# srndpty/kobato-eyes

Hardware: AMD Instinct MI355X
Metric: images/s (pHash + all-pairs Hamming scan + cluster membership) (higher is better)
Workload: dtype u8 luma, int32 taps (i8 matrix cores), f64 DCT, 1-bit Hamming products (fp4 matrix cores, exact)

## Files before the change

### kobato-eyes_amd/csrc/ke_api.hip

```cpp
#include <cstdarg>
#include <cstdio>
#include <algorithm>
#include <cmath>
#include <numeric>
#include <unordered_map>

#include <fcntl.h>
#include <sys/stat.h>
#include <unistd.h>

#include "ke_internal.h"

static thread_local std::string g_create_err;

int ke_fail(ke_ctx *ctx, int code, const char *fmt, ...) {
    char msg[512];
    va_list ap;
    va_start(ap, fmt);
    vsnprintf(msg, sizeof msg, fmt, ap);
    va_end(ap);
    if (ctx)
        ctx->err = msg;
    else
        g_create_err = msg;
// ... 129 lines not shown
        delete t;
        return nullptr;
    }
    c->mx[key] = t;
    return t;
}

void ke_time_begin(ke_ctx *ctx, int kind) {
    ctx->ev_valid[kind] = false;
    (void)hipEventRecord(ctx->ev0[kind], ctx->stream);
}

void ke_time_end(ke_ctx *ctx, int kind) {
    if (hipEventRecord(ctx->ev1[kind], ctx->stream) == hipSuccess) ctx->ev_valid[kind] = true;
}

KE_API int ke_abi_version(void) { return KE_ABI_VERSION; }

KE_API const char *ke_create_error(void) { return g_create_err.c_str(); }

KE_API ke_ctx *ke_create(int device_id) {
    int count = 0;
    if (hipGetDeviceCount(&count) != hipSuccess || count <= 0) {
        ke_fail(nullptr, KE_ENODEV, "no HIP device visible (libkeyes_hip has no CPU fallback)");
        return nullptr;
    }
    if (device_id < 0 || device_id >= count) {
        ke_fail(nullptr, KE_EINVAL, "device_id %d out of range [0,%d)", device_id, count);
        return nullptr;
    }
    if (hipSetDevice(device_id) != hipSuccess) {
        ke_fail(nullptr, KE_EHIP, "hipSetDevice(%d) failed", device_id);
        return nullptr;
    }
    hipDeviceProp_t prop;
    if (hipGetDeviceProperties(&prop, device_id) != hipSuccess) {
        ke_fail(nullptr, KE_EHIP, "hipGetDeviceProperties failed");
        return nullptr;
    }
    if (std::strncmp(prop.gcnArchName, "gfx950", 6) != 0) {
        ke_fail(nullptr, KE_ENODEV, "device %d is %s; this library is built for gfx950 only", device_id,
                prop.gcnArchName);
        return nullptr;
    }
    auto *ctx = new ke_ctx();
    ctx->device = device_id;
    ctx->cu_count = prop.multiProcessorCount;
    if (hipStreamCreateWithFlags(&ctx->own_stream, hipStreamNonBlocking) != hipSuccess) {
        ke_fail(nullptr, KE_EHIP, "hipStreamCreate failed");
        delete ctx;
        return nullptr;
    }
    ctx->stream = ctx->own_stream;
    for (int k = 0; k < KE_T_COUNT; ++k) {
        (void)hipEventCreate(&ctx->ev0[k]);
        (void)hipEventCreate(&ctx->ev1[k]);
    }
    return ctx;
}

static void stage_free(ke_ctx *ctx);

KE_API void ke_destroy(ke_ctx *ctx) {
    if (!ctx) return;
    (void)hipSetDevice(ctx->device);
    (void)hipStreamSynchronize(ctx->stream);
    stage_free(ctx);
    for (int k = 0; k < 2; ++k) {
        if (ctx->side[k]) (void)hipStreamDestroy(ctx->side[k]);
        if (ctx->side_join[k]) (void)hipEventDestroy(ctx->side_join[k]);
    }
    if (ctx->side_fork) (void)hipEventDestroy(ctx->side_fork);
    if (ctx->h_comm) (void)hipHostFree(ctx->h_comm);
    if (ctx->h_meta) (void)hipHostFree(ctx->h_meta);
    for (auto &b : ctx->buf)
        if (b.ptr) (void)hipFree(b.ptr);
    free_coeff_cache(ctx);
    for (int k = 0; k < KE_T_COUNT; ++k) {
        (void)hipEventDestroy(ctx->ev0[k]);
        (void)hipEventDestroy(ctx->ev1[k]);
    }
    (void)hipStreamDestroy(ctx->own_stream);
    delete ctx;
}

KE_API const char *ke_last_error(ke_ctx *ctx) { return ctx ? ctx->err.c_str() : g_create_err.c_str(); }

KE_API int ke_set_stream(ke_ctx *ctx, void *hip_stream) {
    if (!ctx) return KE_EINVAL;
    ctx->stream = hip_stream ? (hipStream_t)hip_stream : ctx->own_stream;
    return KE_OK;
}

KE_API void *ke_get_stream(ke_ctx *ctx) { return ctx ? (void *)ctx->stream : nullptr; }

KE_API int ke_synchronize(ke_ctx *ctx) {
    if (!ctx) return KE_EINVAL;
    KE_HIP(ctx, hipStreamSynchronize(ctx->stream));
    return KE_OK;
}

KE_API int ke_device_info(ke_ctx *ctx, char *name, size_t name_len, int32_t *compute_units, int64_t *total_mem) {
    if (!ctx) return KE_EINVAL;
    hipDeviceProp_t prop;
    KE_HIP(ctx, hipGetDeviceProperties(&prop, ctx->device));
    if (name && name_len) std::snprintf(name, name_len, "%s (%s)", prop.name, prop.gcnArchName);
    if (compute_units) *compute_units = prop.multiProcessorCount;
    if (total_mem) *total_mem = (int64_t)prop.totalGlobalMem;
    return KE_OK;
}

KE_API int ke_malloc(ke_ctx *ctx, size_t bytes, void **out) {
    if (!ctx || !out) return KE_EINVAL;
    KE_HIP(ctx, hipMalloc(out, bytes ? bytes : 16));
    return KE_OK;
}

KE_API int ke_free(ke_ctx *ctx, void *p) {
    if (!ctx) return KE_EINVAL;
    KE_HIP(ctx, hipStreamSynchronize(ctx->stream));
    KE_HIP(ctx, hipFree(p));
    return KE_OK;
}

KE_API int ke_host_alloc(ke_ctx *ctx, size_t bytes, void **out) {
    if (!ctx || !out) return KE_EINVAL;
    KE_HIP(ctx, hipSetDevice(ctx->device));
// ... 485 lines not shown
        }
        cursor += 2 * idx.size();
    }
    if (used) KE_HIP(ctx, hipMemcpyAsync(s.d_px, s.h_px, used, hipMemcpyHostToDevice, st->copy_stream));
    if (cursor) KE_HIP(ctx, hipMemcpyAsync(s.d_meta, s.h_meta, cursor * 8, hipMemcpyHostToDevice, st->copy_stream));
    KE_HIP(ctx, hipEventRecord(s.copied, st->copy_stream));
    KE_HIP(ctx, hipStreamWaitEvent(ctx->stream, s.copied, 0));
    if (phash_out) KE_HIP(ctx, hipMemsetAsync(s.d_ph, 0, (size_t)n * 8, ctx->stream));
    if (dhash_out) KE_HIP(ctx, hipMemsetAsync(s.d_dh, 0, (size_t)n * 8, ctx->stream));
    if (margin_out) KE_HIP(ctx, hipMemsetAsync(s.d_mg, 0, (size_t)n * 4, ctx->stream));
    MarginScope margin_scope{ctx};
    ctx->margin_cur = margin_out ? s.d_mg : nullptr;
    ke_time_begin(ctx, KE_T_HASH);
    size_t gi = 0;
    for (auto &kv : groups) {
        const int w = std::get<0>(kv.first), h = std::get<1>(kv.first), c = std::get<2>(kv.first);
        const uint64_t *d_off = s.d_meta + spans[gi].first;
        const int64_t m = (int64_t)spans[gi].second;
        KeHashGroup g{s.d_px, d_off, (uint64_t)w * h * c, (const int64_t *)(d_off + m), m, w, h, c};
        for (int64_t idx : kv.second)
            if (((uintptr_t)s.d_px + offsets[idx]) % 4 != 0) { g.misaligned = true; break; }
        KE_TRY(ke_launch_hash_group(ctx, g, phash_out ? s.d_ph : nullptr, dhash_out ? s.d_dh : nullptr, nullptr, nullptr));
        ++gi;
    }
    ke_time_end(ctx, KE_T_HASH);
    if (phash_out) KE_HIP(ctx, hipMemcpyAsync(s.h_ph, s.d_ph, (size_t)n * 8, hipMemcpyDeviceToHost, ctx->stream));
    if (dhash_out) KE_HIP(ctx, hipMemcpyAsync(s.h_dh, s.d_dh, (size_t)n * 8, hipMemcpyDeviceToHost, ctx->stream));
    if (margin_out) KE_HIP(ctx, hipMemcpyAsync(s.h_mg, s.d_mg, (size_t)n * 4, hipMemcpyDeviceToHost, ctx->stream));
    KE_HIP(ctx, hipEventRecord(s.done, ctx->stream));
    s.user_ph = phash_out; s.user_dh = dhash_out; s.user_mg = margin_out; s.n = n;
    s.in_flight = true;
    return KE_OK;
}

KE_API int ke_hamming_scan(ke_ctx *ctx, const uint64_t *hashes, const int64_t *ids, const int64_t *sizes, int64_t n,
                           int32_t part_index, int32_t part_count, int32_t threshold, int32_t band_bits,
                           int32_t band_count, double size_ratio, int64_t bucket_pair_cap, ke_edge *edges_out,
                           int64_t capacity, int64_t *n_edges_out, uint64_t *counters_out) {
    if (!ctx) return KE_EINVAL;
    if (n < 0 || (n > 0 && !hashes)) return ke_fail(ctx, KE_EINVAL, "hashes is NULL");
    if (!n_edges_out) return ke_fail(ctx, KE_EINVAL, "n_edges_out is NULL");
    if (band_bits <= 0) return ke_fail(ctx, KE_EINVAL, "band_bits must be positive");
    if (band_count <= 0) return ke_fail(ctx, KE_EINVAL, "band_count must be positive");
    if ((int64_t)band_bits * band_count > 64) return ke_fail(ctx, KE_EINVAL, "band config too large");
    if (threshold < 0 || threshold > 64) return ke_fail(ctx, KE_EINVAL, "hamming_threshold must be in [0, 64]");
    if (part_count <= 0 || part_index < 0 || part_index >= part_count)
        return ke_fail(ctx, KE_EINVAL, "bad shard %d/%d", part_index, part_count);
    if (capacity < 0 || (capacity > 0 && !edges_out)) return ke_fail(ctx, KE_EINVAL, "edges_out is NULL");
    *n_edges_out = 0;
    if (counters_out) std::memset(counters_out, 0, 4 * sizeof(uint64_t));
    if (n < 2) return KE_OK;
    KE_HIP(ctx, hipSetDevice(ctx->device));
    const void *d_h, *d_ids, *d_sizes;
    const bool any_host = !ke_is_device_ptr(hashes) || (ids && !ke_is_device_ptr(ids)) || (sizes && !ke_is_device_ptr(sizes));
    if (any_host) {
        void *base;
        KE_TRY(ke_reserve(ctx, KE_BUF_SCAN_IN, (size_t)n * 24, &base));
        auto stage = [&](const void *src, size_t slot, const void **dst) -> int {
            if (!src) { *dst = nullptr; return KE_OK; }
            if (ke_is_device_ptr(src)) { *dst = src; return KE_OK; }
            void *d = (uint8_t *)base + slot * (size_t)n * 8;
            KE_HIP(ctx, hipMemcpyAsync(d, src, (size_t)n * 8, hipMemcpyHostToDevice, ctx->stream));
            *dst = d;
            return KE_OK;
        };
        KE_TRY(stage(hashes, 0, &d_h));
        KE_TRY(stage(ids, 1, &d_ids));
        KE_TRY(stage(sizes, 2, &d_sizes));
    } else {
        d_h = hashes; d_ids = ids; d_sizes = sizes;
    }
    const bool edges_dev = capacity > 0 && ke_is_device_ptr(edges_out);
    ke_edge *d_edges = edges_out;
    void *tmp;
    if (capacity > 0 && !edges_dev) {
        KE_TRY(ke_reserve(ctx, KE_BUF_SCAN_EDGES, (size_t)capacity * sizeof(ke_edge), &tmp));
        d_edges = (ke_edge *)tmp;
    }
    KE_TRY(ke_reserve(ctx, KE_BUF_SCAN_CNT, 4 * sizeof(unsigned long long), &tmp));
    unsigned long long *d_cnt = (unsigned long long *)tmp;
    KE_HIP(ctx, hipMemsetAsync(d_cnt, 0, 4 * sizeof(unsigned long long), ctx->stream));
    unsigned long long pairs = 0;
    KE_TRY(ke_launch_scan(ctx, (const uint64_t *)d_h, (const int64_t *)d_ids, (const int64_t *)d_sizes, n, part_index,
                          part_count, threshold, band_bits, band_count, size_ratio, bucket_pair_cap, d_edges, capacity,
                          d_cnt, &pairs, counters_out != nullptr));
    unsigned long long h_cnt[4];
    KE_HIP(ctx, hipMemcpyAsync(h_cnt, d_cnt, sizeof h_cnt, hipMemcpyDeviceToHost, ctx->stream));
    KE_HIP(ctx, hipStreamSynchronize(ctx->stream));
    *n_edges_out = (int64_t)h_cnt[2];
    if (h_cnt[0] != pairs)
        return ke_fail(ctx, KE_EHIP, "scan evaluated %llu pairs, expected %llu", h_cnt[0], pairs);
    if (counters_out)
        for (int k = 0; k < 4; ++k) counters_out[k] = h_cnt[k];
    if (capacity > 0 && !edges_dev) {
        const int64_t m = std::min<int64_t>(capacity, (int64_t)h_cnt[2]);
        if (m > 0) {
            KE_HIP(ctx, hipMemcpyAsync(edges_out, d_edges, (size_t)m * sizeof(ke_edge), hipMemcpyDeviceToHost, ctx->stream));
            KE_HIP(ctx, hipStreamSynchronize(ctx->stream));
        }
    }
    return KE_OK;
}

KE_API int ke_band_pairs_after_size(ke_ctx *ctx, const uint64_t *hashes, const int64_t *sizes, int64_t n, int32_t band_bits,
                                    int32_t band_count, double size_ratio, int64_t bucket_pair_cap, uint64_t *count_out) {
    if (!ctx) return KE_EINVAL;
    if (!count_out) return ke_fail(ctx, KE_EINVAL, "count_out is NULL");
    if (n < 0 || (n > 0 && (!hashes || !sizes))) return ke_fail(ctx, KE_EINVAL, "hashes / sizes is NULL");
    if (band_bits <= 0 || band_count <= 0 || (int64_t)band_bits * band_count > 64) return ke_fail(ctx, KE_EINVAL, "bad band config");
    if (!(size_ratio > 0.0)) return ke_fail(ctx, KE_EINVAL, "size_ratio must be positive (without a size filter the counter equals the bucket pairs)");
    *count_out = 0;
    if (n < 2) return KE_OK;
    KE_HIP(ctx, hipSetDevice(ctx->device));
    const void *d_h = hashes, *d_s = sizes;
    if (!ke_is_device_ptr(hashes) || !ke_is_device_ptr(sizes)) {
        void *base;
        KE_TRY(ke_reserve(ctx, KE_BUF_SCAN_IN, (size_t)n * 24, &base));
        if (!ke_is_device_ptr(hashes)) {
            KE_HIP(ctx, hipMemcpyAsync(base, hashes, (size_t)n * 8, hipMemcpyHostToDevice, ctx->stream));
            d_h = base;
        }
        if (!ke_is_device_ptr(sizes)) {
            void *d = (uint8_t *)base + (size_t)n * 16;
            KE_HIP(ctx, hipMemcpyAsync(d, sizes, (size_t)n * 8, hipMemcpyHostToDevice, ctx->stream));
            d_s = d;
        }
    }
    void *tmp;
    KE_TRY(ke_reserve(ctx, KE_BUF_SCAN_CNT, 4 * sizeof(unsigned long long), &tmp));
    unsigned long long *d_cnt = (unsigned long long *)tmp;
    KE_HIP(ctx, hipMemsetAsync(d_cnt, 0, sizeof(unsigned long long), ctx->stream));
    KE_TRY(ke_launch_band_pairs_after_size(ctx, (const uint64_t *)d_h, (const int64_t *)d_s, n, band_bits, band_count, size_ratio,
                                           bucket_pair_cap, d_cnt));
    unsigned long long h = 0;
    KE_HIP(ctx, hipMemcpyAsync(&h, d_cnt, sizeof h, hipMemcpyDeviceToHost, ctx->stream));
    KE_HIP(ctx, hipStreamSynchronize(ctx->stream));
    *count_out = h;
    return KE_OK;
}

// ... 312 lines not shown
```

### kobato-eyes_amd/csrc/ke_internal.h

```cpp
#pragma once

#include <hip/hip_runtime.h>

#include <cstdint>
#include <cstring>
#include <map>
#include <string>
#include <thread>
#include <tuple>
#include <utility>
#include <vector>

#include "../../include/keyes.h"

#define KE_API extern "C" __attribute__((visibility("default")))

struct KeAxisCoeffs {
    int in_size = 0, out_size = 0;
    int ksize = 0;
    std::vector<int32_t> bounds;
    std::vector<int32_t> kk;
    int ndw = 0;
    int span = 0;
    std::vector<int32_t> start;
// ... 41 lines not shown
    KE_BUF_SCAN_IN,
    KE_BUF_SCAN_AUX,
    KE_BUF_SCAN_EDGES,
    KE_BUF_SCAN_CNT,
    KE_BUF_SCAN_HIST,
    KE_BUF_SCAN_EXP,
    KE_BUF_SSIM_IN,
    KE_BUF_SSIM_AUX,
    KE_BUF_COMM,
    KE_BUF_COMM_EDGES,
    KE_BUF_JPEG_TABLES,
    KE_BUF_COUNT
};

constexpr int KE_MAX_STAGE_SLOTS = 4;
struct KeStageSlot {
    uint8_t *h_px = nullptr, *d_px = nullptr;
    uint64_t *h_meta = nullptr, *d_meta = nullptr;
    uint64_t *h_ph = nullptr, *h_dh = nullptr, *d_ph = nullptr, *d_dh = nullptr;
    float *h_mg = nullptr, *d_mg = nullptr;
    hipEvent_t copied = nullptr, done = nullptr;
    bool in_flight = false;
    bool px_external = false;
    uint64_t *user_ph = nullptr, *user_dh = nullptr;
    float *user_mg = nullptr;
    int64_t n = 0;
};
struct KeStage {
    size_t bytes = 0;
    int64_t max_images = 0;
    int n_slots = 0, next = 0;
    hipStream_t copy_stream = nullptr;
    KeStageSlot slot[KE_MAX_STAGE_SLOTS];
};

struct ke_ctx {
    int device = 0;
    int cu_count = 0;
    hipStream_t own_stream = nullptr;
    hipStream_t stream = nullptr;
    std::string err;
    KeDevBuf buf[KE_BUF_COUNT];
    std::map<std::tuple<int, int, uint32_t, uint32_t>, KeAxisCoeffs *> coeffs;
    hipEvent_t ev0[KE_T_COUNT] = {}, ev1[KE_T_COUNT] = {};
    bool ev_valid[KE_T_COUNT] = {};
    KeStage *stage = nullptr;
    hipStream_t side[2] = {nullptr, nullptr};
    hipEvent_t side_fork = nullptr, side_join[2] = {nullptr, nullptr};
    int64_t edge_slots = 1024;
    void *h_comm = nullptr;
    size_t h_comm_bytes = 0;
    void *h_meta = nullptr;
    size_t h_meta_bytes = 0;
    bool ssim_exact = false;
    float *margin_cur = nullptr;
    bool dct_tables_ready = false;
};

int ke_fail(ke_ctx *ctx, int code, const char *fmt, ...);
#define KE_HIP(ctx, call)                                                                        \
    do {                                                                                         \
        hipError_t e_ = (call);                                                                  \
        if (e_ != hipSuccess)                                                                    \
            return ke_fail((ctx), KE_EHIP, "%s failed: %s (%s:%d)", #call, hipGetErrorString(e_), \
                           __FILE__, __LINE__);                                                  \
    } while (0)
#define KE_TRY(expr)            \
    do {                        \
        int rc_ = (expr);       \
        if (rc_ != KE_OK) return rc_; \
    } while (0)

bool ke_is_device_ptr(const void *p);
int ke_reserve(ke_ctx *ctx, int which, size_t bytes, void **out);
int ke_to_device(ke_ctx *ctx, const void *p, size_t bytes, int which, const void **dev);
const KeAxisCoeffs *ke_get_coeffs(ke_ctx *ctx, int in_size, int out_size, int filter = KE_FILTER_LANCZOS, float in0 = 0.0f,
                                  float in1 = -1.0f);
const KeChunkTable *ke_get_chunks(ke_ctx *ctx, const KeAxisCoeffs *c, int cpo, int ndwc_multiple = 4);
const KeMxTable *ke_get_mx(ke_ctx *ctx, const KeAxisCoeffs *c, int min_ks = 0, bool align64 = false);
void ke_time_begin(ke_ctx *ctx, int kind);
void ke_time_end(ke_ctx *ctx, int kind);

struct KeHashGroup {
    const uint8_t *pixels;
    const uint64_t *offsets;
    uint64_t stride;
    const int64_t *out_idx;
    int64_t n;
    int w, h, channels;
    bool misaligned = false;
};
int ke_launch_hash_group(ke_ctx *ctx, const KeHashGroup &g, uint64_t *d_phash, uint64_t *d_dhash,
                         uint8_t *d_tile32_out, uint8_t *d_tile98_out, hipStream_t fused_stream = nullptr);
int ke_launch_resize_group(ke_ctx *ctx, const KeHashGroup &g, int ow, int oh, int filter, uint8_t *d_tiles,
                           const float *box = nullptr);
int ke_launch_tile_ahash(ke_ctx *ctx, const uint8_t *d_tiles, int64_t n, int grid, int tile, uint64_t *d_bits);
int ke_launch_sad_pairs(ke_ctx *ctx, const uint8_t *d_thumbs, int64_t pixels, const int64_t *d_pa, const int64_t *d_pb,
                        int64_t n_pairs, uint64_t *d_out);
int ke_launch_band_pairs_after_size(ke_ctx *ctx, const uint64_t *d_hashes, const int64_t *d_sizes, int64_t n, int band_bits,
                                    int band_count, double ratio, int64_t bucket_pair_cap, unsigned long long *d_out);
int ke_launch_scan(ke_ctx *ctx, const uint64_t *d_hashes, const int64_t *d_ids, const int64_t *d_sizes, int64_t n,
                   int part_index, int part_count, int threshold, int band_bits, int band_count, double size_ratio,
                   int64_t bucket_pair_cap, ke_edge *d_edges, int64_t capacity, unsigned long long *d_counters,
                   unsigned long long *pairs_evaluated, bool want_bucket_pairs);
int ke_launch_ssim(ke_ctx *ctx, const uint8_t *d_images, int w, int h, int channels, const int64_t *d_pa,
                   const int64_t *d_pb, int64_t n_pairs, double *d_out);
// ... 16 lines not shown
```

### kobato-eyes_amd/csrc/ke_scan.hip

```cpp
#include <cmath>

#include <hipcub/hipcub.hpp>

#include "ke_internal.h"

namespace {

constexpr int kThreads = 512;
constexpr int kRT = 8;
constexpr int kTile = 8 * kRT * 16;
constexpr int kCols = 1024;
constexpr int kCPR = kTile / kCols;
constexpr int kChunk = 256;

typedef int ke_v8i __attribute__((ext_vector_type(8)));
typedef int ke_v4i __attribute__((ext_vector_type(4)));
typedef float ke_v4f __attribute__((ext_vector_type(4)));

struct ScanArgs {
    const uint64_t *hashes;
    const ke_v4i *expanded;
    const int64_t *ids;
    const int64_t *sizes;
    int64_t n;
    int nb;
    int ncc;
    int64_t first_tile;
    int64_t tile_step;
    int64_t n_tiles;
    int threshold, band_bits, band_count;
    double size_ratio;
    const uint32_t *hist;
    const uint32_t *blen;
    unsigned long long cap;
    ke_edge *edges;
    int64_t capacity;
    unsigned long long *counters;
    int xcd_remap;
};

__device__ __forceinline__ int popc64(uint32_t lo, uint32_t hi) { return __popc(lo) + __popc(hi); }

__device__ void consider_pair(const ScanArgs &a, int64_t gi, int64_t gj, uint64_t x, uint64_t y, int pc) {
    if (gi >= gj || gj >= a.n) return;
    if (a.ids && a.ids[gi] == a.ids[gj]) return;
    if (a.sizes && a.size_ratio > 0.0) {
        const int64_t sa = a.sizes[gi], sb = a.sizes[gj];
        if (sa > 0 && sb > 0) {
            const int64_t small = sa < sb ? sa : sb, large = sa < sb ? sb : sa;
            if (!((double)small / (double)large >= a.size_ratio)) return;
        }
    }
    const uint64_t d = x ^ y;
    const uint64_t mask = a.band_bits >= 64 ? ~0ull : ((1ull << a.band_bits) - 1ull);
    int bands = 0, shared = 0;
    for (int b = 0; b < a.band_count; ++b) {
        const int sh = b * a.band_bits;
        if (((d >> sh) & mask) != 0) continue;
        if (a.cap) {
            const unsigned long long len = a.hist ? a.hist[((size_t)b << a.band_bits) + (size_t)((x >> sh) & mask)]
                                                  : a.blen[(size_t)b * (size_t)a.n + (size_t)gi];
            if (len * (len - 1) / 2 > a.cap) continue;
        }
        bands |= 1 << (b < 31 ? b : 31);
        ++shared;
    }
    if (!shared) return;
    atomicAdd(&a.counters[1], (unsigned long long)shared);
    const unsigned long long slot = atomicAdd(&a.counters[2], 1ull);
    if ((int64_t)slot < a.capacity) {
        ke_edge e;
        e.a = gi; e.b = gj; e.h = pc; e.bands = bands;
        a.edges[slot] = e;
    }
}

__device__ __forceinline__ uint32_t spread8(uint32_t b) {
    uint32_t t = (b | (b << 12)) & 0x000F000Fu;
    t = (t | (t << 6)) & 0x03030303u;
    t = (t | (t << 3)) & 0x11111111u;
    return t << 1;
}

__global__ __launch_bounds__(256) void ke_scan_expand(const uint64_t *__restrict__ hashes, int64_t n, int64_t n_pad,
                                                       ke_v4i *__restrict__ out) {
    const int64_t e = (int64_t)blockIdx.x * 256 + threadIdx.x;
    if (e >= n_pad * 4) return;
    const int64_t i = (e >> 6) * 16 + (e & 15);
    const int g = (int)(e >> 4) & 3;
    ke_v4i v = {0, 0, 0, 0};
    if (i < n) {
        const uint64_t x = g < 2 ? hashes[i] : ~hashes[i];
        const uint32_t half = (uint32_t)(x >> (32 * (g & 1)));
#pragma unroll
        for (int k = 0; k < 4; ++k) v[k] = (int)spread8((half >> (8 * k)) & 0xFFu);
    }
    out[e] = v;
}

__global__ __launch_bounds__(kThreads) void ke_scan_tiles(const ScanArgs a) {
    __shared__ ke_v4i s_b[2][kChunk / 16 * 64];
    const int tid = threadIdx.x, lane = tid & 63, wv = tid >> 6;
    int64_t slot = blockIdx.x;
    if (a.xcd_remap) {
        const int64_t per = ((int64_t)gridDim.x + 7) / 8;
        slot = (int64_t)(blockIdx.x & 7) * per + (blockIdx.x >> 3);
        if (slot >= (int64_t)gridDim.x) return;
    }
    const int64_t t = a.first_tile + slot * a.tile_step;
    if (t >= a.n_tiles) return;
    const double hc = 0.5 * kCPR, bq = (double)a.ncc + hc;
    int64_t rb = (int64_t)floor((bq - sqrt(fmax(bq * bq - 4.0 * hc * (double)t, 0.0))) / (2.0 * hc));
    if (rb < 0) rb = 0;
    if (rb >= a.nb) rb = a.nb - 1;
    while (rb > 0 && rb * a.ncc - kCPR * rb * (rb - 1) / 2 > t) --rb;
    while (rb + 1 < a.nb && (rb + 1) * a.ncc - kCPR * (rb + 1) * rb / 2 <= t) ++rb;
    const int64_t cc = kCPR * rb + (t - (rb * a.ncc - kCPR * rb * (rb - 1) / 2));
    const int64_t row0 = rb * kTile, col0 = cc * kCols;
    const int64_t wrow0 = row0 + (int64_t)wv * (kRT * 16);
    if (tid == 0) {
        const int64_t rows = min((int64_t)kTile, a.n - row0), cols = min((int64_t)kCols, a.n - col0);
        const unsigned long long pairs = cc == kCPR * rb ? (unsigned long long)(rows * (rows - 1) / 2) : (unsigned long long)(rows * cols);
        atomicAdd(&a.counters[0], pairs);
    }

    ke_v8i ra[kRT];
#pragma unroll
    for (int r = 0; r < kRT; ++r) {
        const ke_v4i v = a.expanded[(wrow0 / 16 + r) * 64 + lane];
        ra[r] = ke_v8i{v[0], v[1], v[2], v[3], 0, 0, 0, 0};
    }
    const int thr_bits = __float_as_int((float)(64 - a.threshold));
    const int nchunks = (int)((min((int64_t)kCols, a.n - col0) + kChunk - 1) / kChunk);
    const ke_v4i *cbase = a.expanded + (col0 / 16) * 64;
    ke_v4i pre0 = cbase[tid], pre1 = cbase[kThreads + tid];
    s_b[0][tid] = pre0;
    s_b[0][kThreads + tid] = pre1;
    __builtin_amdgcn_s_waitcnt(0x0F70);
    __syncthreads();
    for (int c = 0; c < nchunks; ++c) {
        {
            const int cn = c + 1 < nchunks ? c + 1 : c;
            pre0 = cbase[cn * (kChunk / 16 * 64) + tid];
            pre1 = cbase[cn * (kChunk / 16 * 64) + kThreads + tid];
        }
        const ke_v4i *bt = s_b[c & 1];
        const int64_t below = wrow0 - (col0 + (int64_t)c * kChunk) - 15;
        const int ct0 = below < 0 ? 0 : (int)min((int64_t)(kChunk / 16), below / 16 + 1);
        for (int ct = ct0; ct < kChunk / 16; ++ct) {
            const ke_v4i bv = bt[ct * 64 + lane];
            const ke_v8i b = {bv[0], bv[1], bv[2], bv[3], 0, 0, 0, 0};
            ke_v4f acc[kRT];
#pragma unroll
            for (int r = 0; r < kRT; ++r)
                acc[r] = __builtin_amdgcn_mfma_scale_f32_16x16x128_f8f6f4(ra[r], b, ke_v4f{0, 0, 0, 0}, 4, 4, 0, 0, 0, 0);
            int m = 0;
#pragma unroll
            for (int r = 0; r < kRT; ++r) {
                m = max(max(m, __float_as_int(acc[r][0])), __float_as_int(acc[r][1]));
                m = max(max(m, __float_as_int(acc[r][2])), __float_as_int(acc[r][3]));
            }
            if (__ballot(m >= thr_bits) != 0ull) {
                uint32_t hits = 0;
#pragma unroll
                for (int r = 0; r < kRT; ++r)
#pragma unroll
                    for (int i = 0; i < 4; ++i) hits |= __float_as_int(acc[r][i]) >= thr_bits ? 1u << (4 * r + i) : 0u;
                const int64_t gj = col0 + (int64_t)c * kChunk + ct * 16 + (lane & 15);
                if (gj >= a.n) hits = 0;
                const uint64_t y = hits ? a.hashes[gj] : 0ull;
                while (hits) {
                    const int k = __ffs(hits) - 1;
                    hits &= hits - 1;
                    const int64_t gi = wrow0 + (k >> 2) * 16 + 4 * (lane >> 4) + (k & 3);
                    if (gi < gj) {
                        const uint64_t x = a.hashes[gi];
                        consider_pair(a, gi, gj, x, y, __popcll(x ^ y));
                    }
                }
            }
        }
        s_b[(c + 1) & 1][tid] = pre0;
        s_b[(c + 1) & 1][kThreads + tid] = pre1;
        __syncthreads();
    }
}

__global__ void ke_band_hist(const uint64_t *__restrict__ hashes, int64_t n, int band_bits, int band_count,
                             uint32_t *__restrict__ hist) {
    const int64_t i = (int64_t)blockIdx.x * blockDim.x + threadIdx.x;
    if (i >= n) return;
    const uint64_t x = hashes[i];
    const uint64_t mask = (1ull << band_bits) - 1ull;
    for (int b = 0; b < band_count; ++b) atomicAdd(&hist[((size_t)b << band_bits) + (size_t)((x >> (b * band_bits)) & mask)], 1u);
}

__global__ void ke_hist_pairs(const uint32_t *__restrict__ hist, size_t bins, unsigned long long cap, unsigned long long *out) {
    unsigned long long s = 0;
    for (size_t i = (size_t)blockIdx.x * blockDim.x + threadIdx.x; i < bins; i += (size_t)gridDim.x * blockDim.x) {
        const unsigned long long len = hist[i];
        const unsigned long long p = len * (len - 1) / 2;
        if (len >= 2 && (!cap || p <= cap)) s += p;
    }
    for (int d = 32; d > 0; d >>= 1) s += __shfl_down(s, d);
    __shared__ unsigned long long part[4];
    if ((threadIdx.x & 63) == 0) part[threadIdx.x >> 6] = s;
    __syncthreads();
    if (threadIdx.x == 0 && (part[0] | part[1] | part[2] | part[3])) atomicAdd(out, part[0] + part[1] + part[2] + part[3]);
}

__global__ void ke_band_keys(const uint64_t *__restrict__ hashes, int64_t n, int shift, uint64_t mask, uint64_t *__restrict__ keys,
                             uint32_t *__restrict__ pos) {
    const int64_t i = (int64_t)blockIdx.x * blockDim.x + threadIdx.x;
    if (i >= n) return;
    keys[i] = (hashes[i] >> shift) & mask;
    pos[i] = (uint32_t)i;
}

__global__ void ke_run_lengths(const uint64_t *__restrict__ keys, const uint32_t *__restrict__ pos, int64_t n, unsigned long long cap,
                               uint32_t *__restrict__ blen, unsigned long long *out) {
    const int64_t i = (int64_t)blockIdx.x * blockDim.x + threadIdx.x;
    if (i >= n) return;
    if (i > 0 && keys[i - 1] == keys[i]) return;
    int64_t e = i + 1;
    while (e < n && keys[e] == keys[i]) ++e;
    const unsigned long long len = (unsigned long long)(e - i);
    for (int64_t k = i; k < e; ++k) blen[pos[k]] = (uint32_t)len;
    const unsigned long long p = len * (len - 1) / 2;
    if (len >= 2 && (!cap || p <= cap)) atomicAdd(out, p);
}

__global__ void ke_size_keys(const int64_t *__restrict__ sizes, int64_t n, uint64_t *__restrict__ keys, uint32_t *__restrict__ pos) {
    const int64_t i = (int64_t)blockIdx.x * blockDim.x + threadIdx.x;
    if (i >= n) return;
    const int64_t s = sizes[i];
    keys[i] = s > 0 ? (uint64_t)s : 0ull;
    pos[i] = (uint32_t)i;
}

__global__ void ke_band_keys_of(const uint64_t *__restrict__ hashes, const uint32_t *__restrict__ order, int64_t n, int shift,
                                uint64_t mask, uint64_t *__restrict__ keys) {
    const int64_t i = (int64_t)blockIdx.x * blockDim.x + threadIdx.x;
    if (i < n) keys[i] = (hashes[order[i]] >> shift) & mask;
}

__global__ void ke_run_flags(const uint64_t *__restrict__ keys, int64_t n, uint32_t *__restrict__ flags) {
    const int64_t i = (int64_t)blockIdx.x * blockDim.x + threadIdx.x;
// ... 49 lines not shown
    KE_HIP(ctx, hipcub::DeviceRadixSort::SortPairs(nullptr, t_size, (const uint64_t *)nullptr, (uint64_t *)nullptr,
                                                   (const uint32_t *)nullptr, (uint32_t *)nullptr, (int)n, 0, 64, ctx->stream));
    KE_HIP(ctx, hipcub::DeviceRadixSort::SortPairs(nullptr, t_band, (const uint64_t *)nullptr, (uint64_t *)nullptr,
                                                   (const uint64_t *)nullptr, (uint64_t *)nullptr, (int)n, 0, band_bits, ctx->stream));
    KE_HIP(ctx, hipcub::DeviceScan::InclusiveSum(nullptr, t_scan, (const uint32_t *)nullptr, (uint32_t *)nullptr, (int)n, ctx->stream));
    const size_t temp_bytes = std::max(t_size, std::max(t_band, t_scan));
    const size_t kb = ((size_t)n * 8 + 255) & ~(size_t)255, pb = ((size_t)(n + 1) * 4 + 255) & ~(size_t)255;
    void *scratch;
    KE_TRY(ke_reserve(ctx, KE_BUF_SCAN_AUX, 4 * kb + 4 * pb + temp_bytes + 256, &scratch));
    uint8_t *sp = (uint8_t *)scratch;
    uint64_t *k_a = (uint64_t *)sp, *k_b = (uint64_t *)(sp + kb), *sz_sorted = (uint64_t *)(sp + 2 * kb), *sz_band = (uint64_t *)(sp + 3 * kb);
    uint32_t *p_a = (uint32_t *)(sp + 4 * kb), *order = (uint32_t *)(sp + 4 * kb + pb), *rank1 = (uint32_t *)(sp + 4 * kb + 2 * pb),
             *starts = (uint32_t *)(sp + 4 * kb + 3 * pb);
    void *temp = sp + 4 * kb + 4 * pb;
    const dim3 grid((unsigned)((n + 255) / 256)), blk(256);
    const uint64_t mask = band_bits >= 64 ? ~0ull : ((1ull << band_bits) - 1ull);
    hipLaunchKernelGGL(ke_size_keys, grid, blk, 0, ctx->stream, d_sizes, n, k_a, p_a);
    size_t tb = temp_bytes;
    KE_HIP(ctx, hipcub::DeviceRadixSort::SortPairs(temp, tb, (const uint64_t *)k_a, sz_sorted, (const uint32_t *)p_a, order, (int)n, 0, 64, ctx->stream));
    for (int b = 0; b < band_count; ++b) {
        hipLaunchKernelGGL(ke_band_keys_of, grid, blk, 0, ctx->stream, d_hashes, (const uint32_t *)order, n, b * band_bits, mask, k_a);
        tb = temp_bytes;
        KE_HIP(ctx, hipcub::DeviceRadixSort::SortPairs(temp, tb, (const uint64_t *)k_a, k_b, (const uint64_t *)sz_sorted, sz_band, (int)n, 0,
                                                       band_bits, ctx->stream));
        uint32_t *flags = p_a;
        hipLaunchKernelGGL(ke_run_flags, grid, blk, 0, ctx->stream, (const uint64_t *)k_b, n, flags);
        tb = temp_bytes;
        KE_HIP(ctx, hipcub::DeviceScan::InclusiveSum(temp, tb, (const uint32_t *)flags, rank1, (int)n, ctx->stream));
        hipLaunchKernelGGL(ke_run_starts, grid, blk, 0, ctx->stream, (const uint64_t *)k_b, (const uint32_t *)rank1, n, starts);
        hipLaunchKernelGGL(ke_size_pairs, grid, blk, 0, ctx->stream, (const uint64_t *)sz_band, (const uint32_t *)rank1,
                           (const uint32_t *)starts, n, ratio, cap, d_out);
        KE_HIP(ctx, hipGetLastError());
    }
    return KE_OK;
}

int ke_launch_scan(ke_ctx *ctx, const uint64_t *d_hashes, const int64_t *d_ids, const int64_t *d_sizes, int64_t n,
                   int part_index, int part_count, int threshold, int band_bits, int band_count, double size_ratio,
                   int64_t bucket_pair_cap, ke_edge *d_edges, int64_t capacity, unsigned long long *d_counters,
                   unsigned long long *pairs_evaluated, bool want_bucket_pairs) {
    ScanArgs a;
    a.hashes = d_hashes; a.ids = d_ids; a.sizes = (size_ratio > 0.0) ? d_sizes : nullptr;
    a.n = n;
    a.nb = (int)((n + kTile - 1) / kTile);
    a.ncc = (int)((n + kCols - 1) / kCols);
    a.n_tiles = (int64_t)a.nb * a.ncc - (int64_t)kCPR * a.nb * (a.nb - 1) / 2;
    a.first_tile = part_index;
    a.tile_step = part_count;
    a.threshold = threshold; a.band_bits = band_bits; a.band_count = band_count;
    a.size_ratio = size_ratio;
    a.hist = nullptr; a.blen = nullptr;
    a.cap = bucket_pair_cap > 0 ? (unsigned long long)bucket_pair_cap : 0ull;
    a.edges = d_edges; a.capacity = capacity; a.counters = d_counters;
    if ((bucket_pair_cap > 0 || want_bucket_pairs) && band_bits <= 24) {
        void *h;
        const size_t bins = (size_t)band_count << band_bits, bytes = bins * sizeof(uint32_t);
        KE_TRY(ke_reserve(ctx, KE_BUF_SCAN_HIST, bytes, &h));
        KE_HIP(ctx, hipMemsetAsync(h, 0, bytes, ctx->stream));
        hipLaunchKernelGGL(ke_band_hist, dim3((unsigned)((n + 255) / 256)), dim3(256), 0, ctx->stream, d_hashes, n, band_bits,
                           band_count, (uint32_t *)h);
        KE_HIP(ctx, hipGetLastError());
        a.hist = (const uint32_t *)h;
        if (want_bucket_pairs) {
            const unsigned blocks = (unsigned)std::min<size_t>((bins + 1023) / 1024, 256);
            hipLaunchKernelGGL(ke_hist_pairs, dim3(blocks), dim3(256), 0, ctx->stream, (const uint32_t *)h, bins, a.cap, d_counters + 3);
            KE_HIP(ctx, hipGetLastError());
        }
    } else if (bucket_pair_cap > 0 || want_bucket_pairs) {
        if (n > 0xffffffffLL) return ke_fail(ctx, KE_EUNSUPPORTED, "bands wider than 24 bits need n < 2^32");
        size_t temp_bytes = 0;
        KE_HIP(ctx, hipcub::DeviceRadixSort::SortPairs(nullptr, temp_bytes, (const uint64_t *)nullptr, (uint64_t *)nullptr,
                                                       (const uint32_t *)nullptr, (uint32_t *)nullptr, (int)n, 0, band_bits, ctx->stream));
        const size_t kb = ((size_t)n * 8 + 255) & ~(size_t)255, pb = ((size_t)n * 4 + 255) & ~(size_t)255;
        void *scratch, *lens;
        KE_TRY(ke_reserve(ctx, KE_BUF_SCAN_AUX, 2 * kb + 2 * pb + temp_bytes + 256, &scratch));
        KE_TRY(ke_reserve(ctx, KE_BUF_SCAN_HIST, (size_t)band_count * n * sizeof(uint32_t), &lens));
        uint8_t *sp = (uint8_t *)scratch;
        uint64_t *k_in = (uint64_t *)sp, *k_out = (uint64_t *)(sp + kb);
        uint32_t *p_in = (uint32_t *)(sp + 2 * kb), *p_out = (uint32_t *)(sp + 2 * kb + pb);
        void *temp = sp + 2 * kb + 2 * pb;
        const uint64_t mask = band_bits >= 64 ? ~0ull : ((1ull << band_bits) - 1ull);
        const dim3 grid((unsigned)((n + 255) / 256)), blk(256);
        for (int b = 0; b < band_count; ++b) {
            hipLaunchKernelGGL(ke_band_keys, grid, blk, 0, ctx->stream, d_hashes, n, b * band_bits, mask, k_in, p_in);
            KE_HIP(ctx, hipcub::DeviceRadixSort::SortPairs(temp, temp_bytes, k_in, k_out, p_in, p_out, (int)n, 0, band_bits, ctx->stream));
            hipLaunchKernelGGL(ke_run_lengths, grid, blk, 0, ctx->stream, k_out, p_out, n, a.cap, (uint32_t *)lens + (size_t)b * n,
                               want_bucket_pairs ? d_counters + 3 : d_counters + 3);
            KE_HIP(ctx, hipGetLastError());
        }
        a.blen = (const uint32_t *)lens;
    }
    const int64_t my_tiles = a.n_tiles > part_index ? (a.n_tiles - part_index + part_count - 1) / part_count : 0;
    const int64_t n_pad = (int64_t)a.nb * kTile;
    void *exp;
    KE_TRY(ke_reserve(ctx, KE_BUF_SCAN_EXP, (size_t)n_pad * 64, &exp));
    a.expanded = (const ke_v4i *)exp;
    ke_time_begin(ctx, KE_T_SCAN);
    if (my_tiles > 0) {
        hipLaunchKernelGGL(ke_scan_expand, dim3((unsigned)((n_pad * 4 + 255) / 256)), dim3(256), 0, ctx->stream, d_hashes, n, n_pad,
                           (ke_v4i *)exp);
        if (my_tiles > 0x7fffffffLL) return ke_fail(ctx, KE_EUNSUPPORTED, "too many tiles for one launch");
        static const int xcd = [] { const char *e = std::getenv("KE_SCAN_XCD"); return e ? std::atoi(e) : 0; }();
        a.xcd_remap = xcd;
        const int64_t grid = xcd ? (my_tiles + 7) / 8 * 8 : my_tiles;
        hipLaunchKernelGGL(ke_scan_tiles, dim3((unsigned)grid), dim3(kThreads), 0, ctx->stream, a);
        KE_HIP(ctx, hipGetLastError());
    }
    ke_time_end(ctx, KE_T_SCAN);
    unsigned long long pairs = 0;
    for (int64_t rb = 0; rb < a.nb; ++rb) {
        const int64_t off = rb * a.ncc - (int64_t)kCPR * rb * (rb - 1) / 2;
        const int64_t row0 = rb * kTile, rows = std::min<int64_t>(kTile, n - row0);
        for (int64_t cc = kCPR * rb; cc < a.ncc; ++cc) {
            const int64_t t = off + (cc - kCPR * rb);
            const bool diagonal = cc < kCPR * (rb + 1);
            if (!diagonal) {
                const int64_t last = a.ncc - 1;
                const int64_t t_last = off + (last - kCPR * rb);
                const int64_t first_full_t = t, end_full_t = t_last;
                if (end_full_t > first_full_t) {
                    auto upto = [&](int64_t x) { return x <= part_index ? 0 : (x - part_index + part_count - 1) / part_count; };
                    pairs += (unsigned long long)(upto(end_full_t) - upto(first_full_t)) * (unsigned long long)(rows * kCols);
                }
                if (t_last % part_count == part_index && last >= cc)
                    pairs += (unsigned long long)(rows * std::min<int64_t>(kCols, n - last * kCols));
                break;
            }
            if (t % part_count != part_index) continue;
            const int64_t col0 = cc * kCols, cols = std::min<int64_t>(kCols, n - col0);
            for (int64_t j = col0; j < col0 + cols; ++j)
                pairs += (unsigned long long)std::max<int64_t>(0, std::min<int64_t>(rows, j - row0));
        }
    }
    *pairs_evaluated = pairs;
    return KE_OK;
}
```

Baseline: 8.599 million.

## Switch Hamming scan to 32x32 fp4 MFMA with half-size expanded hashes

Re-encodes hash bits so that a single fp4 MFMA over 64 bits yields the Hamming distance directly, via an offset/bias encoding. This removes the separate complemented operand and halves the expanded-hash buffer. The scan now uses 32x32x64 MFMA tiles (4 row tiles of 32) instead of 16x16x128, with one prefetch per thread per chunk. The band histogram build and counter clearing are folded into the expand kernel, which drops a memset and a launch. A pinned host counter block replaces the stack readback, and a bias template variant handles thresholds of 32 and above, which adds some risk to correctness of the threshold encoding.

```diff
diff --git a/kobato-eyes_amd/csrc/ke_api.hip b/kobato-eyes_amd/csrc/ke_api.hip
--- a/kobato-eyes_amd/csrc/ke_api.hip
+++ b/kobato-eyes_amd/csrc/ke_api.hip
@@ -205,6 +205,12 @@
         return nullptr;
     }
     ctx->stream = ctx->own_stream;
+    if (hipHostMalloc((void **)&ctx->h_words, 8 * sizeof(unsigned long long), hipHostMallocDefault) != hipSuccess) {
+        ke_fail(nullptr, KE_EHIP, "hipHostMalloc of the counter block failed");
+        (void)hipStreamDestroy(ctx->own_stream);
+        delete ctx;
+        return nullptr;
+    }
     for (int k = 0; k < KE_T_COUNT; ++k) {
         (void)hipEventCreate(&ctx->ev0[k]);
         (void)hipEventCreate(&ctx->ev1[k]);
@@ -226,6 +232,7 @@
     if (ctx->side_fork) (void)hipEventDestroy(ctx->side_fork);
     if (ctx->h_comm) (void)hipHostFree(ctx->h_comm);
     if (ctx->h_meta) (void)hipHostFree(ctx->h_meta);
+    if (ctx->h_words) (void)hipHostFree(ctx->h_words);
     for (auto &b : ctx->buf)
         if (b.ptr) (void)hipFree(b.ptr);
     free_coeff_cache(ctx);
@@ -817,23 +824,20 @@
     if (n < 2) return KE_OK;
     KE_HIP(ctx, hipSetDevice(ctx->device));
     const void *d_h, *d_ids, *d_sizes;
-    const bool any_host = !ke_is_device_ptr(hashes) || (ids && !ke_is_device_ptr(ids)) || (sizes && !ke_is_device_ptr(sizes));
-    if (any_host) {
+    const bool h_dev = ke_is_device_ptr(hashes), i_dev = !ids || ke_is_device_ptr(ids), s_dev = !sizes || ke_is_device_ptr(sizes);
+    d_h = hashes; d_ids = ids; d_sizes = sizes;
+    if (!h_dev || !i_dev || !s_dev) {
         void *base;
         KE_TRY(ke_reserve(ctx, KE_BUF_SCAN_IN, (size_t)n * 24, &base));
         auto stage = [&](const void *src, size_t slot, const void **dst) -> int {
-            if (!src) { *dst = nullptr; return KE_OK; }
-            if (ke_is_device_ptr(src)) { *dst = src; return KE_OK; }
             void *d = (uint8_t *)base + slot * (size_t)n * 8;
             KE_HIP(ctx, hipMemcpyAsync(d, src, (size_t)n * 8, hipMemcpyHostToDevice, ctx->stream));
             *dst = d;
             return KE_OK;
         };
-        KE_TRY(stage(hashes, 0, &d_h));
-        KE_TRY(stage(ids, 1, &d_ids));
-        KE_TRY(stage(sizes, 2, &d_sizes));
-    } else {
-        d_h = hashes; d_ids = ids; d_sizes = sizes;
+        if (!h_dev) KE_TRY(stage(hashes, 0, &d_h));
+        if (!i_dev) KE_TRY(stage(ids, 1, &d_ids));
+        if (!s_dev) KE_TRY(stage(sizes, 2, &d_sizes));
     }
     const bool edges_dev = capacity > 0 && ke_is_device_ptr(edges_out);
     ke_edge *d_edges = edges_out;
@@ -844,13 +848,12 @@
     }
     KE_TRY(ke_reserve(ctx, KE_BUF_SCAN_CNT, 4 * sizeof(unsigned long long), &tmp));
     unsigned long long *d_cnt = (unsigned long long *)tmp;
-    KE_HIP(ctx, hipMemsetAsync(d_cnt, 0, 4 * sizeof(unsigned long long), ctx->stream));
     unsigned long long pairs = 0;
     KE_TRY(ke_launch_scan(ctx, (const uint64_t *)d_h, (const int64_t *)d_ids, (const int64_t *)d_sizes, n, part_index,
                           part_count, threshold, band_bits, band_count, size_ratio, bucket_pair_cap, d_edges, capacity,
                           d_cnt, &pairs, counters_out != nullptr));
-    unsigned long long h_cnt[4];
-    KE_HIP(ctx, hipMemcpyAsync(h_cnt, d_cnt, sizeof h_cnt, hipMemcpyDeviceToHost, ctx->stream));
+    unsigned long long *h_cnt = ctx->h_words;
+    KE_HIP(ctx, hipMemcpyAsync(h_cnt, d_cnt, 4 * sizeof(unsigned long long), hipMemcpyDeviceToHost, ctx->stream));
     KE_HIP(ctx, hipStreamSynchronize(ctx->stream));
     *n_edges_out = (int64_t)h_cnt[2];
     if (h_cnt[0] != pairs)
diff --git a/kobato-eyes_amd/csrc/ke_internal.h b/kobato-eyes_amd/csrc/ke_internal.h
--- a/kobato-eyes_amd/csrc/ke_internal.h
+++ b/kobato-eyes_amd/csrc/ke_internal.h
@@ -117,6 +117,7 @@
     size_t h_comm_bytes = 0;
     void *h_meta = nullptr;
     size_t h_meta_bytes = 0;
+    unsigned long long *h_words = nullptr;
     bool ssim_exact = false;
     float *margin_cur = nullptr;
     bool dct_tables_ready = false;
diff --git a/kobato-eyes_amd/csrc/ke_scan.hip b/kobato-eyes_amd/csrc/ke_scan.hip
--- a/kobato-eyes_amd/csrc/ke_scan.hip
+++ b/kobato-eyes_amd/csrc/ke_scan.hip
@@ -7,15 +7,16 @@
 namespace {
 
 constexpr int kThreads = 512;
-constexpr int kRT = 8;
-constexpr int kTile = 8 * kRT * 16;
+constexpr int kRT = 4;
+constexpr int kOT = 32;
+constexpr int kTile = 8 * kRT * kOT;
 constexpr int kCols = 1024;
 constexpr int kCPR = kTile / kCols;
 constexpr int kChunk = 256;
 
 typedef int ke_v8i __attribute__((ext_vector_type(8)));
 typedef int ke_v4i __attribute__((ext_vector_type(4)));
-typedef float ke_v4f __attribute__((ext_vector_type(4)));
+typedef float ke_v16f __attribute__((ext_vector_type(16)));
 
 struct ScanArgs {
     const uint64_t *hashes;
@@ -79,27 +80,34 @@
     uint32_t t = (b | (b << 12)) & 0x000F000Fu;
     t = (t | (t << 6)) & 0x03030303u;
     t = (t | (t << 3)) & 0x11111111u;
-    return t << 1;
-}
-
-__global__ __launch_bounds__(256) void ke_scan_expand(const uint64_t *__restrict__ hashes, int64_t n, int64_t n_pad,
-                                                       ke_v4i *__restrict__ out) {
+    return (t << 3) | 0x22222222u;
+}
+
+__global__ __launch_bounds__(256) void ke_scan_prepare(const uint64_t *__restrict__ hashes, int64_t n, int64_t n_pad,
+                                                        ke_v4i *__restrict__ out, int band_bits, int band_count,
+                                                        uint32_t *__restrict__ hist, unsigned long long *__restrict__ counters,
+                                                        int clear_counters) {
     const int64_t e = (int64_t)blockIdx.x * 256 + threadIdx.x;
-    if (e >= n_pad * 4) return;
-    const int64_t i = (e >> 6) * 16 + (e & 15);
-    const int g = (int)(e >> 4) & 3;
+    if (e < 4 && clear_counters) counters[e] = 0ull;
+    if (e >= n_pad * 2) return;
+    const int64_t i = (e >> 6) * kOT + (e & 31);
     ke_v4i v = {0, 0, 0, 0};
     if (i < n) {
-        const uint64_t x = g < 2 ? hashes[i] : ~hashes[i];
-        const uint32_t half = (uint32_t)(x >> (32 * (g & 1)));
+        const uint32_t half = (uint32_t)(hashes[i] >> (32 * ((int)(e >> 5) & 1)));
 #pragma unroll
         for (int k = 0; k < 4; ++k) v[k] = (int)spread8((half >> (8 * k)) & 0xFFu);
     }
     out[e] = v;
-}
-
+    if (hist && e < n) {
+        const uint64_t x = hashes[e];
+        const uint64_t mask = (1ull << band_bits) - 1ull;
+        for (int b = 0; b < band_count; ++b) atomicAdd(&hist[((size_t)b << band_bits) + (size_t)((x >> (b * band_bits)) & mask)], 1u);
+    }
+}
+
+template <bool kBias>
 __global__ __launch_bounds__(kThreads) void ke_scan_tiles(const ScanArgs a) {
-    __shared__ ke_v4i s_b[2][kChunk / 16 * 64];
+    __shared__ ke_v4i s_b[2][kChunk / kOT * 64];
     const int tid = threadIdx.x, lane = tid & 63, wv = tid >> 6;
     int64_t slot = blockIdx.x;
     if (a.xcd_remap) {
@@ -117,7 +125,7 @@
     while (rb + 1 < a.nb && (rb + 1) * a.ncc - kCPR * (rb + 1) * rb / 2 <= t) ++rb;
     const int64_t cc = kCPR * rb + (t - (rb * a.ncc - kCPR * rb * (rb - 1) / 2));
     const int64_t row0 = rb * kTile, col0 = cc * kCols;
-    const int64_t wrow0 = row0 + (int64_t)wv * (kRT * 16);
+    const int64_t wrow0 = row0 + (int64_t)wv * (kRT * kOT);
     if (tid == 0) {
         const int64_t rows = min((int64_t)kTile, a.n - row0), cols = min((int64_t)kCols, a.n - col0);
         const unsigned long long pairs = cc == kCPR * rb ? (unsigned long long)(rows * (rows - 1) / 2) : (unsigned long long)(rows * cols);
@@ -127,52 +135,56 @@
     ke_v8i ra[kRT];
 #pragma unroll
     for (int r = 0; r < kRT; ++r) {
-        const ke_v4i v = a.expanded[(wrow0 / 16 + r) * 64 + lane];
+        const ke_v4i v = a.expanded[(wrow0 / kOT + r) * 64 + lane];
         ra[r] = ke_v8i{v[0], v[1], v[2], v[3], 0, 0, 0, 0};
     }
-    const int thr_bits = __float_as_int((float)(64 - a.threshold));
+    constexpr float kStart = kBias ? 65.0f : 0.0f;
+    const int thr_bits = __float_as_int(kStart + (float)(64 - 2 * a.threshold));
     const int nchunks = (int)((min((int64_t)kCols, a.n - col0) + kChunk - 1) / kChunk);
-    const ke_v4i *cbase = a.expanded + (col0 / 16) * 64;
-    ke_v4i pre0 = cbase[tid], pre1 = cbase[kThreads + tid];
-    s_b[0][tid] = pre0;
-    s_b[0][kThreads + tid] = pre1;
+    constexpr int kPieces = kChunk / kOT * 64;
+    static_assert(kPieces == kThreads, "one piece of a column chunk per thread");
+    const ke_v4i *cbase = a.expanded + (col0 / kOT) * 64;
+    ke_v4i pre = cbase[tid];
+    s_b[0][tid] = pre;
     __builtin_amdgcn_s_waitcnt(0x0F70);
     __syncthreads();
     for (int c = 0; c < nchunks; ++c) {
         {
             const int cn = c + 1 < nchunks ? c + 1 : c;
-            pre0 = cbase[cn * (kChunk / 16 * 64) + tid];
-            pre1 = cbase[cn * (kChunk / 16 * 64) + kThreads + tid];
+            pre = cbase[cn * kPieces + tid];
         }
         const ke_v4i *bt = s_b[c & 1];
-        const int64_t below = wrow0 - (col0 + (int64_t)c * kChunk) - 15;
-        const int ct0 = below < 0 ? 0 : (int)min((int64_t)(kChunk / 16), below / 16 + 1);
-        for (int ct = ct0; ct < kChunk / 16; ++ct) {
+        const int64_t below = wrow0 - (col0 + (int64_t)c * kChunk) - (kOT - 1);
+        const int ct0 = below < 0 ? 0 : (int)min((int64_t)(kChunk / kOT), below / kOT + 1);
+        for (int ct = ct0; ct < kChunk / kOT; ++ct) {
             const ke_v4i bv = bt[ct * 64 + lane];
             const ke_v8i b = {bv[0], bv[1], bv[2], bv[3], 0, 0, 0, 0};
-            ke_v4f acc[kRT];
+            ke_v16f acc[kRT];
+#pragma unroll
+            for (int r = 0; r < kRT; ++r) {
+                ke_v16f c0;
+#pragma unroll
+                for (int i = 0; i < 16; ++i) c0[i] = kStart;
+                acc[r] = __builtin_amdgcn_mfma_scale_f32_32x32x64_f8f6f4(ra[r], b, c0, 4, 4, 0, 0, 0, 0);
+            }
+            int m = 0;
 #pragma unroll
             for (int r = 0; r < kRT; ++r)
-                acc[r] = __builtin_amdgcn_mfma_scale_f32_16x16x128_f8f6f4(ra[r], b, ke_v4f{0, 0, 0, 0}, 4, 4, 0, 0, 0, 0);
-            int m = 0;
-#pragma unroll
-            for (int r = 0; r < kRT; ++r) {
-                m = max(max(m, __float_as_int(acc[r][0])), __float_as_int(acc[r][1]));
-                m = max(max(m, __float_as_int(acc[r][2])), __float_as_int(acc[r][3]));
-            }
+#pragma unroll
+                for (int i = 0; i < 16; i += 2) m = max(max(m, __float_as_int(acc[r][i])), __float_as_int(acc[r][i + 1]));
             if (__ballot(m >= thr_bits) != 0ull) {
-                uint32_t hits = 0;
+                uint64_t hits = 0;
 #pragma unroll
                 for (int r = 0; r < kRT; ++r)
 #pragma unroll
-                    for (int i = 0; i < 4; ++i) hits |= __float_as_int(acc[r][i]) >= thr_bits ? 1u << (4 * r + i) : 0u;
-                const int64_t gj = col0 + (int64_t)c * kChunk + ct * 16 + (lane & 15);
+                    for (int i = 0; i < 16; ++i) hits |= __float_as_int(acc[r][i]) >= thr_bits ? 1ull << (16 * r + i) : 0ull;
+                const int64_t gj = col0 + (int64_t)c * kChunk + ct * kOT + (lane & 31);
                 if (gj >= a.n) hits = 0;
                 const uint64_t y = hits ? a.hashes[gj] : 0ull;
                 while (hits) {
-                    const int k = __ffs(hits) - 1;
+                    const int k = __ffsll((unsigned long long)hits) - 1;
                     hits &= hits - 1;
-                    const int64_t gi = wrow0 + (k >> 2) * 16 + 4 * (lane >> 4) + (k & 3);
+                    const int64_t gi = wrow0 + (k >> 4) * kOT + (k & 3) + 8 * ((k & 15) >> 2) + 4 * (lane >> 5);
                     if (gi < gj) {
                         const uint64_t x = a.hashes[gi];
                         consider_pair(a, gi, gj, x, y, __popcll(x ^ y));
@@ -180,19 +192,9 @@
                 }
             }
         }
-        s_b[(c + 1) & 1][tid] = pre0;
-        s_b[(c + 1) & 1][kThreads + tid] = pre1;
+        s_b[(c + 1) & 1][tid] = pre;
         __syncthreads();
     }
-}
-
-__global__ void ke_band_hist(const uint64_t *__restrict__ hashes, int64_t n, int band_bits, int band_count,
-                             uint32_t *__restrict__ hist) {
-    const int64_t i = (int64_t)blockIdx.x * blockDim.x + threadIdx.x;
-    if (i >= n) return;
-    const uint64_t x = hashes[i];
-    const uint64_t mask = (1ull << band_bits) - 1ull;
-    for (int b = 0; b < band_count; ++b) atomicAdd(&hist[((size_t)b << band_bits) + (size_t)((x >> (b * band_bits)) & mask)], 1u);
 }
 
 __global__ void ke_hist_pairs(const uint32_t *__restrict__ hist, size_t bins, unsigned long long cap, unsigned long long *out) {
@@ -348,22 +350,20 @@
     a.hist = nullptr; a.blen = nullptr;
     a.cap = bucket_pair_cap > 0 ? (unsigned long long)bucket_pair_cap : 0ull;
     a.edges = d_edges; a.capacity = capacity; a.counters = d_counters;
+    uint32_t *hist = nullptr;
+    size_t bins = 0;
+    bool counters_cleared = false;
     if ((bucket_pair_cap > 0 || want_bucket_pairs) && band_bits <= 24) {
         void *h;
-        const size_t bins = (size_t)band_count << band_bits, bytes = bins * sizeof(uint32_t);
-        KE_TRY(ke_reserve(ctx, KE_BUF_SCAN_HIST, bytes, &h));
-        KE_HIP(ctx, hipMemsetAsync(h, 0, bytes, ctx->stream));
-        hipLaunchKernelGGL(ke_band_hist, dim3((unsigned)((n + 255) / 256)), dim3(256), 0, ctx->stream, d_hashes, n, band_bits,
-                           band_count, (uint32_t *)h);
-        KE_HIP(ctx, hipGetLastError());
-        a.hist = (const uint32_t *)h;
-        if (want_bucket_pairs) {
-            const unsigned blocks = (unsigned)std::min<size_t>((bins + 1023) / 1024, 256);
-            hipLaunchKernelGGL(ke_hist_pairs, dim3(blocks), dim3(256), 0, ctx->stream, (const uint32_t *)h, bins, a.cap, d_counters + 3);
-            KE_HIP(ctx, hipGetLastError());
-        }
+        bins = (size_t)band_count << band_bits;
+        KE_TRY(ke_reserve(ctx, KE_BUF_SCAN_HIST, bins * sizeof(uint32_t), &h));
+        KE_HIP(ctx, hipMemsetAsync(h, 0, bins * sizeof(uint32_t), ctx->stream));
+        hist = (uint32_t *)h;
+        a.hist = hist;
     } else if (bucket_pair_cap > 0 || want_bucket_pairs) {
         if (n > 0xffffffffLL) return ke_fail(ctx, KE_EUNSUPPORTED, "bands wider than 24 bits need n < 2^32");
+        KE_HIP(ctx, hipMemsetAsync(d_counters, 0, 4 * sizeof(unsigned long long), ctx->stream));
+        counters_cleared = true;
         size_t temp_bytes = 0;
         KE_HIP(ctx, hipcub::DeviceRadixSort::SortPairs(nullptr, temp_bytes, (const uint64_t *)nullptr, (uint64_t *)nullptr,
                                                        (const uint32_t *)nullptr, (uint32_t *)nullptr, (int)n, 0, band_bits, ctx->stream));
@@ -389,20 +389,29 @@
     const int64_t my_tiles = a.n_tiles > part_index ? (a.n_tiles - part_index + part_count - 1) / part_count : 0;
     const int64_t n_pad = (int64_t)a.nb * kTile;
     void *exp;
-    KE_TRY(ke_reserve(ctx, KE_BUF_SCAN_EXP, (size_t)n_pad * 64, &exp));
+    KE_TRY(ke_reserve(ctx, KE_BUF_SCAN_EXP, (size_t)n_pad * 32, &exp));
     a.expanded = (const ke_v4i *)exp;
+    if (my_tiles > 0x7fffffffLL) return ke_fail(ctx, KE_EUNSUPPORTED, "too many tiles for one launch");
     ke_time_begin(ctx, KE_T_SCAN);
+    hipLaunchKernelGGL(ke_scan_prepare, dim3((unsigned)((n_pad * 2 + 255) / 256)), dim3(256), 0, ctx->stream, d_hashes, n, n_pad,
+                       (ke_v4i *)exp, band_bits, band_count, hist, d_counters, counters_cleared ? 0 : 1);
+    KE_HIP(ctx, hipGetLastError());
     if (my_tiles > 0) {
-        hipLaunchKernelGGL(ke_scan_expand, dim3((unsigned)((n_pad * 4 + 255) / 256)), dim3(256), 0, ctx->stream, d_hashes, n, n_pad,
-                           (ke_v4i *)exp);
-        if (my_tiles > 0x7fffffffLL) return ke_fail(ctx, KE_EUNSUPPORTED, "too many tiles for one launch");
         static const int xcd = [] { const char *e = std::getenv("KE_SCAN_XCD"); return e ? std::atoi(e) : 0; }();
         a.xcd_remap = xcd;
         const int64_t grid = xcd ? (my_tiles + 7) / 8 * 8 : my_tiles;
-        hipLaunchKernelGGL(ke_scan_tiles, dim3((unsigned)grid), dim3(kThreads), 0, ctx->stream, a);
+        if (threshold < 32)
+            hipLaunchKernelGGL(ke_scan_tiles<false>, dim3((unsigned)grid), dim3(kThreads), 0, ctx->stream, a);
+        else
+            hipLaunchKernelGGL(ke_scan_tiles<true>, dim3((unsigned)grid), dim3(kThreads), 0, ctx->stream, a);
         KE_HIP(ctx, hipGetLastError());
     }
     ke_time_end(ctx, KE_T_SCAN);
+    if (hist && want_bucket_pairs) {
+        const unsigned blocks = (unsigned)std::min<size_t>((bins + 1023) / 1024, 256);
+        hipLaunchKernelGGL(ke_hist_pairs, dim3(blocks), dim3(256), 0, ctx->stream, (const uint32_t *)hist, bins, a.cap, d_counters + 3);
+        KE_HIP(ctx, hipGetLastError());
+    }
     unsigned long long pairs = 0;
     for (int64_t rb = 0; rb < a.nb; ++rb) {
         const int64_t off = rb * a.ncc - (int64_t)kCPR * rb * (rb - 1) / 2;
```

After: 8.655 million (median of 6 runs). No clear change (+0.6%).
